# jacklu2016/or-gym-inventory

Measured on AMD Instinct MI355X. Metric: env-steps/sec (batched) at 1/2/4/8 MI355X; % HBM roofline, higher is better.
Workload: dtype int64

## Files before the change

or-gym-inventory_amd/csrc/capi.hip:

```cpp
#include <dlfcn.h>
#include <hip/hip_runtime.h>

#include <algorithm>
#include <cmath>
#include <cstdio>
#include <cstdlib>
#include <cstring>
#include <string>
#include <vector>

#include "../../include/invsim.h"
#include "kernels.hpp"

using namespace invsim;

namespace {

thread_local std::string g_last_error;

struct Field {
    std::string name;
    int64_t offset;
    int32_t elem;
    int32_t rows;
// ... 9 lines not shown
hipError_t ptrs_stats_nv_ph(unsigned long long *out, bool clear);
hipError_t ptrs_stats_im(unsigned long long *out, bool clear);
hipError_t ptrs_stats_im_ph(unsigned long long *out, bool clear);
hipError_t ptrs_stats_netspec(unsigned long long *out, bool clear);
hipError_t ptrs_stats_net(unsigned long long *out, bool clear);
#endif
}

struct invsim_handle {
    int32_t family = 0;
    int32_t device = 0;
    int64_t N = 0, Npad = 0;
    int32_t obs_dim = 0, act_dim = 0, demand_dim = 1;
    char *arena = nullptr;
    int64_t arena_bytes = 0;
    char *tables = nullptr;
    void *scratch = nullptr;
    bool la_valid = false;
    int la_slot = 0;
    std::vector<Field> fields;
    Common cm{};
    NvParams nv{};
    ImParams im{};
    NetParams net{};
    int32_t im_m1 = 0;
    bool im_backlog = false;
    int32_t net_spec = 0;
    bool t_known = true;
    int32_t t_cur = 0;
    int32_t horizon = 0;
    bool past_ok = false;
    int32_t demand_stream = INVSIM_DEMAND_NUMPY;
    uint64_t ph_step = 0;
    int64_t o_phstep = 0;
    bool ph_from_blob = false;
    bool capturing = false;
    bool cap_t_known = true, cap_la_valid = false;
    int32_t cap_t_cur = 0;
    int cap_la_slot = 0;
    int64_t cap_steps = 0;
    std::string err;
};

namespace {

struct Roctx {
// ... 207 lines not shown
        if (p && n) std::memcpy(b.data() + off, p, n * sizeof(T));
        return (int64_t)off;
    }
};

template <typename T>
const T *tab(invsim_handle *h, int64_t off) {
    return reinterpret_cast<const T *>(h->tables + off);
}

bool valid_autoreset(int32_t m) { return m >= 0 && m <= 2; }

int finish_create(invsim_handle *h, invsim_handle **out, int rc) {
    if (rc != INVSIM_OK) {
        g_last_error = h->err;
        invsim_destroy(h);
        *out = nullptr;
        return rc;
    }
    *out = h;
    return INVSIM_OK;
}

int64_t pad_n(int64_t n) { return std::max<int64_t>(256, (n + 255) / 256 * 256); }

void rhs_table(PtrsConst &c, std::vector<double> &tab) {
    c.k0 = 0;
    c.nk = 0;
    c.toff = (int32_t)tab.size();
    if (!(c.lam >= 10) || c.lam > 1e8) return;
    const double sd = std::sqrt(c.lam);
    int64_t k0 = std::max<int64_t>(0, (int64_t)std::floor(c.lam - 12 * sd - 10));
    const int64_t k1 = (int64_t)std::ceil(c.lam + 12 * sd + 40);
    int64_t n = k1 - k0;
    if (n > RHS_LDS_MAX) {
        k0 = std::max<int64_t>(0, (int64_t)std::floor(c.lam) - RHS_LDS_MAX / 2 + 20);
        n = RHS_LDS_MAX;
    }
    for (int64_t k = k0; k < k0 + n; k++)
        tab.push_back(-c.lam + (double)k * c.loglam - np_loggam((double)(k + 1)));
    c.k0 = (int32_t)k0;
    c.nk = (int32_t)n;
}

}

extern "C" {
// ... 164 lines not shown
        p.cm = h->cm;
        if (s->dist == 2) p.nd = np_dist_binomial(s->dist_n, s->dist_p);
        if (s->dist == 3) p.nd = np_dist_integers(s->dist_low, s->dist_high);
        if (s->dist == 4) p.nd = np_dist_geometric(s->dist_p);
        p.periods = s->periods;
        p.lt_max = D;
        p.dist = s->dist;
        int off = 0;
        for (int i = 0; i < m1; i++) {
            p.L[i] = (int32_t)s->lead_time[i];
            p.ring_off[i] = off;
            off += p.L[i];
            p.c[i] = s->supply_capacity[i];
            p.I0[i] = s->I0[i];
        }
        for (int j = 0; j < m; j++) {
            p.up[j] = (double)s->unit_price[j];
            p.uc[j] = (double)s->unit_cost[j];
            p.hc[j] = (double)s->holding_cost[j];
            p.kc[j] = (double)s->demand_cost[j];
        }
        p.pc = pc;
        p.alpha_pow = tab<double>(h, o_ap);
        p.user_D = tab<int64_t>(h, o_ud);
        p.I = at<int64_t>(h, o_I);
        p.B = at<int64_t>(h, o_B);
        p.Rring = at<int64_t>(h, o_R);
        p.alog = at<int64_t>(h, o_A);
        p.alog32 = at<uint32_t>(h, o_A32);
        p.ahead = nullptr;
        if (s->dist >= 1 && s->dist <= 4) {
            hipError_t e = hipMalloc(&h->scratch, (size_t)(2 * 4 * h->Npad * sizeof(uint64_t)));
            if (e != hipSuccess) rc = fail(h, INVSIM_ENOMEM, "hipMalloc(lookahead cache)");
            else p.ahead = static_cast<uint64_t *>(h->scratch);
        }
        if (rc == INVSIM_OK) rc = init_period(h, s->periods);
    }
    return finish_create(h, out, rc);
}

int invsim_create_netinvmgmt(const invsim_netinvmgmt_spec *s, int64_t n, int32_t device, int32_t ar,
                             invsim_handle **out) {
    if (!s || !out) return fail(nullptr, INVSIM_EINVAL, "null argument");
    if (n < 0 || n > (int64_t)1 << 31) return fail(nullptr, INVSIM_EINVAL, "n_envs out of range");
    if (!valid_autoreset(ar)) return fail(nullptr, INVSIM_EINVAL, "bad autoreset mode");
    const int J = s->n_main, E = s->n_reorder, RL = s->n_retail;
// ... 369 lines not shown
        for (int k = 0; k < K; k++) {
            if (t >= h->horizon && h->cm.autoreset == AR_DISABLED && !h->past_ok)
                return fail(h, INVSIM_ERANGE, "step past the episode horizon with autoreset disabled; reset first");
            t = next_period(t, h->horizon, h->cm.autoreset, h->past_ok);
        }
    }
    if (h->demand_stream == INVSIM_DEMAND_PHILOX) {
        int rc = ph_counter_sync(h, s);
        if (rc != INVSIM_OK) return rc;
    }
    if (h->cm.ep_ret && h->N && !reward)
        return fail(h, INVSIM_EINVAL, "the episode sink folds the reward outputs: pass reward / terminated / truncated");
    bool sunk = false;
    hipError_t e = hipSuccess;
    switch (h->family) {
        case INVSIM_NEWSVENDOR: {
            StepIO<float, float> io{K, (const float *)actions, (float *)obs, reward, terminated, truncated, (float *)final_obs};
            e = nv_run_launch(h->nv, t_u, pol, io, h->la_valid, h->la_slot, s);
            break;
        }
        case INVSIM_INVMGMT: {
            StepIO<int64_t, int64_t> io{K, (const int64_t *)actions, (int64_t *)obs, reward, terminated, truncated,
                                        (int64_t *)final_obs};
            e = im_run_launch(h->im, h->im_m1, h->im_backlog, t_u, pol, io, h->la_valid, h->la_slot, sunk, s);
            break;
        }
        case INVSIM_NETINVMGMT: {
            StepIO<float, float> io{K, (const float *)actions, (float *)obs, reward, terminated, truncated, (float *)final_obs};
            e = h->net_spec ? net_spec_launch(h->net_spec, h->net, t_u, pol, io, h->la_valid, h->la_slot, s)
                            : net_run_launch(h->net, t_u, pol, io, s);
            break;
        }
        default: return fail(h, INVSIM_EINVAL, "bad handle family");
    }
    if (e != hipSuccess) {
        h->la_valid = false;
        return hip_fail(h, e, "step launch");
    }
    if (h->cm.ep_ret && !sunk) {
        if (!reward) return fail(h, INVSIM_EINVAL, "the episode sink needs this launch's reward outputs");
        e = episode_fold_groups_launch(reward, terminated, truncated, K, h->N, h->cm.ep_ret, h->cm.ep_part, s);
        if (e != hipSuccess) return hip_fail(h, e, "episode sink fold");
    }
    if (h->demand_stream == INVSIM_DEMAND_PHILOX) h->ph_step += (uint64_t)K;
    if (h->t_known) {
        for (int k = 0; k < K; k++) h->t_cur = next_period(h->t_cur, h->horizon, h->cm.autoreset, h->past_ok);
    } else if (h->cm.autoreset == AR_DISABLED && !h->past_ok) {
// ... 308 lines not shown
```

or-gym-inventory_amd/csrc/invmgmt.hip:

```cpp
#include "kernels.hpp"

namespace invsim {
namespace {

#ifdef INVSIM_TIMING
__device__ uint64_t g_tbuf[TB_WAVES * TB_PROBES];
#endif

constexpr uint32_t IM_WIDE = 0xFFFFFFFFu;

__device__ __forceinline__ int64_t alog_get(const ImParams &P, int64_t idx) {
    const uint32_t v = P.alog32[idx];
    return v == IM_WIDE ? P.alog[idx] : (int64_t)v;
}

constexpr int im_wlane(int m1) { return m1 * (9 < 36 / m1 ? 9 : 36 / m1); }

__device__ __forceinline__ int64_t wrap_add(int64_t a, int64_t b) {
    return (int64_t)((uint64_t)a + (uint64_t)b);
}
__device__ __forceinline__ int64_t wrap_sub(int64_t a, int64_t b) {
    return (int64_t)((uint64_t)a - (uint64_t)b);
}

__device__ __forceinline__ int64_t min_via_f64(int64_t a, int64_t sup) {
    const double x = (double)a, y = (double)sup;
    return (int64_t)((x <= y) ? x : y);
}

// ... 447 lines not shown
    const int64_t S = P.cm.Npad;
    const int O = M1 * (P.lt_max + 1);
#pragma unroll
    for (int i = 0; i < M1; i++) P.I[i * S + e] = P.I0[i];
    if (BACKLOG) {
#pragma unroll
        for (int q = 0; q <= M1; q++) P.B[q * S + e] = 0;
    }
    P.cm.period[e] = 0;
    if (obs) {
        int64_t *orow = obs + e * O;
        for (int q = 0; q < O; q++) orow[q] = (q < M1) ? P.I0[q] : 0;
    }
}

__device__ __forceinline__ void wg_lds_sync() {
    TBAR_T0();
    __builtin_amdgcn_fence(__ATOMIC_RELEASE, "workgroup", "local");
    __builtin_amdgcn_s_barrier();
    __builtin_amdgcn_fence(__ATOMIC_ACQUIRE, "workgroup", "local");
    TBAR_ADD();
}

template <int M1, bool BACKLOG, bool NPD, bool AHEAD, class RG = Pcg>
__global__ void __launch_bounds__(2 * WAVE)
im_split_kernel(ImParams P, int t, StepIO<int64_t, int64_t> io, int cur, int la0, int gla) {
    extern __shared__ __attribute__((aligned(16))) int64_t im_tile[];
    const int64_t N = P.cm.N;
    const int64_t S = P.cm.Npad;
    double *rhs_l = reinterpret_cast<double *>(im_tile + (int64_t)WAVE * M1 * (P.lt_max + 1));
    uint64_t *Acur = P.ahead ? P.ahead + (int64_t)cur * 4 * S : nullptr;
    uint64_t *Anxt = P.ahead ? P.ahead + (int64_t)(cur ^ 1) * 4 * S : nullptr;
    const int64_t udem = P.user_D[t];
    auto stage_table = [&](int lane) {
        TableStage ts;
        ts.dst = rhs_l;
        const bool has_tab = P.pc.nk > 0 && P.dist == 1;
        const double *tsrc = has_tab ? P.rhs : P.alpha_pow;
        const int qm = has_tab ? P.pc.nk - 1 : 0;
#pragma unroll
        for (int u = 0; u < TableStage::NT; u++) ts.v[u] = tsrc[min(lane + u * WAVE, qm)];
        return ts;
    };
    auto draw = [&](auto &g, uint64_t &u32) -> int64_t {
#ifdef INVSIM_ABL_NO_POISSON
        int64_t x = 20 + (int64_t)(g.lo & 3);
        g.next64();
#else
        int64_t x = NPD ? np_demand(g, u32, P.nd) : (P.dist == 5) ? udem : env_poisson(g, P.pc, rhs_l);
#endif
        return x < 0 ? 0 : x;
    };
    constexpr bool DEC = AHEAD;
    const int bid = (int)blockIdx.x;
    TPROBE(0);
    TPROBE_ID();
    if (AHEAD && bid >= la0 && bid < la0 + gla) {
        const int64_t e = (int64_t)(bid - la0) * (2 * WAVE) + threadIdx.x;
        const bool valid = e < N;
        const int64_t ee = valid ? e : N - 1;
        TableStage ts = stage_table((int)(threadIdx.x & (WAVE - 1)));
        if constexpr (RG::kCounter) {
            RG g;
            P.cm.rng.load(ee, g);
            g.set_step(P.cm.ph_step + 1);
            g.sub(0);
            uint64_t u32 = 0;
            ts.flush((int)(threadIdx.x & (WAVE - 1)));
            const int64_t dn = draw(g, u32);
            if (valid) st_store(Anxt + 2 * S + e, (uint64_t)dn);
            return;
        }
        Pcg g;
        g.hi = Acur[ee];
        g.lo = Acur[S + ee];
        g.inc_hi = P.cm.rng.inc_hi[ee];
        g.inc_lo = P.cm.rng.inc_lo[ee];
        uint64_t u32 = NPD ? Acur[3 * S + ee] : 0;
        PtrsJumpLane jt;
        jt.load((int)(threadIdx.x & (WAVE - 1)));
        ts.flush((int)(threadIdx.x & (WAVE - 1)));
        TPROBE(1);
        int64_t dn;
#ifndef INVSIM_ABL_NO_POISSON
        if (!NPD && P.dist == 1 && P.pc.lam >= 10)
            dn = np_poisson_ptrs_compact(
                g, P.pc, RhsTab{rhs_l}, true, jt,
                [](const PtrsConst &c, int) { return c; });
        else
#endif
            dn = draw(g, u32);
        TPROBE(2);
        if (valid) {
            st_store(Anxt + e, g.hi);
            st_store(Anxt + S + e, g.lo);
            st_store(Anxt + 2 * S + e, (uint64_t)dn);
            if (NPD) st_store(Anxt + 3 * S + e, u32);
        }
        TWAIT();
        TPROBE(5);
        return;
    }
    const int lane = threadIdx.x & (WAVE - 1);
    const bool demand_wave = threadIdx.x < WAVE;
    const int64_t e0 = (int64_t)(AHEAD && bid >= la0 ? bid - gla : bid) * WAVE;
    const int64_t e = e0 + lane;
    const bool valid = e < N;
    const int nvalid = (int)((N - e0) < WAVE ? (N - e0) : WAVE);
    const int D = P.lt_max;
    const int O = M1 * (D + 1);
    int64_t *trow = im_tile + (int64_t)lane * O;
    int64_t *w = trow + M1;
    int64_t *dsh = reinterpret_cast<int64_t *>(rhs_l + RHS_LDS_MAX);
    const int t1 = t + 1;
    const int n = D > 0 ? (t1 < D ? t1 : D) : 0;
    const int nw = n > 0 ? (n - 1) * M1 : 0;
    const int64_t tcount = (int64_t)nvalid * O;
    const int64_t thalf = ((tcount / 2) + 1) & ~(int64_t)1;
    constexpr int WL = im_wlane(M1);
    const bool wreg = (D - 1) * M1 <= WL;
    const int slot0 = D > 0 ? (int)((uint32_t)(t1 - n) % (uint32_t)D) : 0;
    auto wrow = [&](int r) -> int64_t {
        int slot = slot0 + r;
        slot = slot >= D ? slot - D : slot;
        return ((int64_t)slot * S + e) * M1;
    };
#ifndef INVSIM_IM_SPLIT_RW
#define INVSIM_IM_SPLIT_RW 6
#endif
    constexpr int RWN = WL / M1;
    constexpr int RW = INVSIM_IM_SPLIT_RW < RWN ? INVSIM_IM_SPLIT_RW : RWN;
    constexpr int WD = (RWN - RW) * M1 > 0 ? (RWN - RW) * M1 : 1;
    const bool wsplit = DEC && wreg && RW < RWN;
    const int u_dyn = wsplit ? RW * M1 : WL;
    const int rmax = nw > 0 ? nw / M1 - 1 : 0;
    if (demand_wave) {
        const int64_t ee = valid ? e : N - 1;
        TableStage ts;
        RG g;
        uint64_t u32 = 0;
        int64_t d = 0;
        if (AHEAD) {
            if (!DEC) d = (int64_t)Acur[2 * S + ee];
        } else {
            ts = stage_table(lane);
            P.cm.rng.load(ee, g);
            g.set_step(P.cm.ph_step);
            g.sub(0);
            if (NPD && !RG::kCounter) u32 = P.cm.u32buf[ee];
        }
        uint32_t wv[WL];
        {
#pragma unroll
            for (int r = 0; r < RWN; r++) {
#ifdef INVSIM_ABL_NO_WINDOW
#pragma unroll
                for (int i = 0; i < M1; i++) wv[r * M1 + i] = (uint32_t)(r + i);
#else
                if (r < RW || !wsplit) {
                    const uint32_t *src = P.alog32 + wrow(r < rmax ? r : rmax);
#pragma unroll
                    for (int i = 0; i < M1; i++) wv[r * M1 + i] = src[i];
                } else {
#pragma unroll
                    for (int i = 0; i < M1; i++) wv[r * M1 + i] = 0;
                }
#endif
            }
        }
        if (!AHEAD) {
            ts.flush(lane);
            d = draw(g, u32);
        }
        if (!DEC) dsh[lane] = d;
        if (D > 0) {
            if (wreg) {
                bool wide = false;
#pragma unroll
                for (int u = 0; u < WL; u++) {
                    if (u < (D - 1) * M1 && !(u >= nw && u < nw + M1) && !(u >= u_dyn && u < nw))
                        w[u] = (u < nw) ? (int64_t)wv[u] : 0;
                    wide |= (u < nw) && (u < u_dyn) && wv[u] == IM_WIDE;
                }
// ... 7 lines not shown
            } else {
                for (int q = 0; q < nw; q++) w[q] = alog_get(P, wrow(q / M1) + q % M1);
                for (int q = n * M1; q < D * M1; q++) w[q] = 0;
            }
        }
        if (!DEC) wg_lds_sync();
        if (DEC) TWAIT();
        TPROBE(6);
        if constexpr (!RG::kCounter) {
            if (!AHEAD && valid) {
                if (Acur) {
                    st_store(Acur + e, g.hi);
                    st_store(Acur + S + e, g.lo);
                    if (NPD) st_store(Acur + 3 * S + e, u32);
                } else {
                    P.cm.rng.store_state(e, g);
                    if (NPD) P.cm.u32buf[e] = u32;
                }
            }
        }
        wg_lds_sync();
        store_tile<(M1 * 11 * WAVE * 8 / 2 + 16 * WAVE - 1) / (16 * WAVE)>(im_tile, io.obs + e0 * O,
                                                                          thalf < tcount ? thalf : tcount, lane);
        if (!AHEAD && Anxt) {
            if constexpr (RG::kCounter) {
                g.set_step(P.cm.ph_step + 1);
                g.sub(0);
                u32 = 0;
            }
            const int64_t dn = draw(g, u32);
            if (valid) {
                if constexpr (!RG::kCounter) {
                    st_store(Anxt + e, g.hi);
                    st_store(Anxt + S + e, g.lo);
                    if (NPD) st_store(Anxt + 3 * S + e, u32);
                }
                st_store(Anxt + 2 * S + e, (uint64_t)dn);
            }
        }
        TWAIT();
        TPROBE(5);
        return;
    }
    TPROBE_AT(3, WAVE);
    const double apow = P.alpha_pow[t];
    const int64_t *arow = io.act + (valid ? e : N - 1) * M1;
    double *const ep_part = P.cm.ep_ret ? P.cm.ep_part + 4 * (e0 / WAVE) : nullptr;
    EpPart epp;
    double ep_r = 0.0;
    if (ep_part) {
        epp.load(ep_part);
        ep_r = P.cm.ep_ret[valid ? e : N - 1];
    }
    int64_t req[M1], arr[M1], I[M1], B[M1 + 1];
    const int64_t d_ahead = DEC ? (int64_t)Acur[2 * S + (valid ? e : N - 1)] : 0;
    uint32_t wd[WD];
    if (wsplit) {
#pragma unroll
        for (int r = RW; r < RWN; r++) {
#ifdef INVSIM_ABL_NO_WINDOW
#pragma unroll
            for (int i = 0; i < M1; i++) wd[(r - RW) * M1 + i] = (uint32_t)(r + i);
#else
            const uint32_t *src = P.alog32 + wrow(r < rmax ? r : rmax);
#pragma unroll
            for (int i = 0; i < M1; i++) wd[(r - RW) * M1 + i] = src[i];
#endif
        }
    }
#pragma unroll
    for (int i = 0; i < M1; i++) req[i] = arow[i];
#pragma unroll
    for (int i = 0; i < M1; i++) {
        const int L = P.L[i];
        const int row = L > 0 ? P.ring_off[i] + (int)((uint32_t)t % (uint32_t)L) : 0;
        arr[i] = P.Rring[(int64_t)row * S + e];
        if (!(L > 0 && t >= L)) arr[i] = 0;
    }
#pragma unroll
    for (int i = 0; i < M1; i++) I[i] = P.I[i * S + e];
#pragma unroll
    for (int q = 0; q <= M1; q++) B[q] = BACKLOG ? P.B[q * S + e] : 0;
    int64_t ordreq[M1], R[M1], Icur[M1];
#pragma unroll
    for (int i = 0; i < M1; i++) req[i] = req[i] > 0 ? req[i] : 0;
#pragma unroll
    for (int i = 0; i < M1; i++) {
        ordreq[i] = wrap_add(req[i], B[i + 1]);
        const int64_t r = ordreq[i] < P.c[i] ? ordreq[i] : P.c[i];
        R[i] = (i + 1 < M1) ? min_via_f64(r, I[i + 1]) : (int64_t)(double)r;
    }
#pragma unroll
    for (int i = 0; i < M1; i++) Icur[i] = wrap_add(I[i], P.L[i] == 0 ? R[i] : arr[i]);
#pragma unroll
    for (int i = 1; i < M1; i++) Icur[i] = wrap_sub(Icur[i], R[i]);
    int64_t Sv[M1 + 1], U[M1 + 1];
#pragma unroll
    for (int i = 0; i < M1; i++) {
        Sv[i + 1] = R[i];
        U[i + 1] = wrap_sub(ordreq[i], R[i]);
    }
    if (!DEC) wg_lds_sync();
    if (DEC) TWAIT();
    TPROBE_AT(1, WAVE);
    const int64_t d = DEC ? d_ahead : dsh[lane];
// ... 45 lines not shown
            const double rev = np_sum<double>(M1 + 1, [&](int q) { return P.up[q] * (double)Sv[q]; });
            const double pro = np_sum<double>(M1 + 1, [&](int q) { return P.uc[q] * (double)Sv[q]; });
            const double hol = np_sum<double>(M1 + 1, [&](int q) {
                const int64_t inv = (q < M1) ? Icur[q] : 0;
                return P.hc[q] * (double)(inv > 0 ? inv : 0);
            });
            const double pen = np_sum<double>(M1 + 1, [&](int q) { return P.kc[q] * (double)U[q]; });
            rr[2 * (M1 + 1) + 0] = __double_as_longlong(profit);
            rr[2 * (M1 + 1) + 1] = __double_as_longlong(rev);
            rr[2 * (M1 + 1) + 2] = __double_as_longlong(pro);
            rr[2 * (M1 + 1) + 3] = __double_as_longlong(hol);
            rr[2 * (M1 + 1) + 4] = __double_as_longlong(pen);
        }
        ImPending<M1> pend;
#pragma unroll
        for (int i = 0; i < M1; i++) {
            pend.R[i] = R[i];
            pend.req[i] = req[i];
        }
        pend.t = t;
        im_flush_pending<M1>(P, pend, e);
        out_store(io.rew + e, reward);
        out_store(io.term + e, (uint8_t)0);
        out_store(io.trunc + e, (uint8_t)(t1 >= P.periods ? 1 : 0));
        if (P.cm.info_demand) P.cm.info_demand[e] = d;
#pragma unroll
        for (int i = 0; i < M1; i++) st_store(P.I + i * S + e, Icur[i]);
        if (BACKLOG) {
#pragma unroll
            for (int q = 0; q <= M1; q++) st_store(P.B + q * S + e, U[q]);
        }
    }
    if (ep_part) {
        EpLane a;
        if (valid) {
            a.r = ep_r;
            a.add(reward, t1 >= P.periods);
            P.cm.ep_ret[e] = a.r;
        }
        epp.flush(ep_part, a, t1 >= P.periods, lane);
    }
    TWAIT();
    TPROBE_AT(4, WAVE);
}

template <int CH, int RD, class RG>
__device__ __forceinline__ void im_stream_loop(const ImParams &P, RG &g, const double *rhs_l, int64_t *dbuf,
                                               int lane, int K, int nb, int t_start) {
    StreamPos<RG> pos(P.cm.ph_step);
    stream_flat_loop<CH, RD, 1>(
        K, nb, t_start, P.periods,
        [&](int j, int, int64_t &d) {
#ifdef INVSIM_ABL_ROLL_NO_DRAW
            d = 20;
            return true;
#else
            pos.at(g, j, 0);
            return np_poisson_try(g, P.pc, rhs_l, d);
#endif
        },
        [&](int slot, int, int64_t d) { dbuf[slot * WAVE + lane] = d < 0 ? 0 : d; });
}

// ... 719 lines not shown
    const bool two = three && g2 && (g3.x % 2) == 0;
    const dim3 g6(g3.x / 2);
    const int sub = p.cm.kn.im_roll_sub >= WAVE ? (int)std::min<int64_t>(p.cm.kn.im_roll_sub / WAVE, g3.x) : (int)g3.x;
#define R_(B, POL)                                                                                                    \
    do {                                                                                                              \
        if (two) hipLaunchKernelGGL((im_roll3o_kernel<1, 5, 10, B, POL, RG, 2>), g6, dim3(6 * WAVE), 2 * G3::lds(POL), s, p, t_u, io, pv); \
        else if (three) hipLaunchKernelGGL((im_roll3o_kernel<1, 5, 10, B, POL, RG>), g3, dim3(3 * WAVE), G3::lds(POL), s, p, t_u, io, pv); \
        else                                                                                                          \
            for (int g0 = 0; g0 < (int)g3.x; g0 += sub)                                                               \
                hipLaunchKernelGGL((im_roll3_kernel<1, 5, 10, B, POL, RG>), dim3(min(sub, (int)g3.x - g0)), dim3(2 * WAVE), \
                                   G::lds(), s, p, t_u, io, pv, g0);                                                  \
    } while (0)
    if (pol) {
        if (backlog) R_(true, true);
        else R_(false, true);
    } else {
        if (backlog) R_(true, false);
        else R_(false, false);
    }
#undef R_
    return hipGetLastError();
}

}

#define IM_DISPATCH(M1V, BL, LAUNCH)                                   \
    switch (M1V) {                                                     \
        case 1: if (BL) LAUNCH(1, true); else LAUNCH(1, false); break; \
        case 2: if (BL) LAUNCH(2, true); else LAUNCH(2, false); break; \
        case 3: if (BL) LAUNCH(3, true); else LAUNCH(3, false); break; \
        case 4: if (BL) LAUNCH(4, true); else LAUNCH(4, false); break; \
        case 5: if (BL) LAUNCH(5, true); else LAUNCH(5, false); break; \
        case 6: if (BL) LAUNCH(6, true); else LAUNCH(6, false); break; \
        case 7: if (BL) LAUNCH(7, true); else LAUNCH(7, false); break; \
        case 8: if (BL) LAUNCH(8, true); else LAUNCH(8, false); break; \
        default: return hipErrorInvalidValue;                          \
    }

#ifdef INVSIM_IM_FAST_TU
hipError_t im_run_launch_ph(const ImParams &p, int M1, bool backlog, int t_u, const PolicyIO *pol,
                            const StepIO<int64_t, int64_t> &io, bool &ahead, int &slot, bool &sunk, hipStream_t s) {
    sunk = im_sink_noop(p, t_u, pol, io);
    if (p.cm.N == 0 || io.K <= 0) return hipSuccess;
    const size_t lds = (size_t)EPW * M1 * (p.lt_max + 1) * sizeof(int64_t) + RHS_LDS_MAX * sizeof(double);
    const dim3 grid(grid_for(p.cm.N, EPW)), block(WAVE);
    PolicyIO none{};
    const PolicyIO &pv = pol ? *pol : none;
    const bool npd = p.dist >= 2 && p.dist <= 4;
    if (im_split_applies(p, t_u, pol, io)) {
        const size_t lds2 = lds + WAVE * sizeof(int64_t);
        ImParams q = p;
        if (!p.cm.kn.im_ahead) q.ahead = nullptr;
        const bool hit = ahead && q.ahead;
        const int gla = hit ? (int)grid_for(p.cm.N, 2 * WAVE) : 0;
        const dim3 grid2(grid.x + gla), block2(2 * WAVE);
        const int cur = slot;
        const int la0 = 0;
#define S_(M, B)                                                                                        \
    do {                                                                                                \
        if (npd) {                                                                                      \
            if (hit) hipLaunchKernelGGL((im_split_kernel<M, B, true, true, PhiloxGen>), grid2, block2, lds2, s, q, t_u, io, cur, la0, gla);  \
            else hipLaunchKernelGGL((im_split_kernel<M, B, true, false, PhiloxGen>), grid2, block2, lds2, s, q, t_u, io, cur, la0, gla);     \
        } else {                                                                                        \
            if (hit) hipLaunchKernelGGL((im_split_kernel<M, B, false, true, PhiloxGen>), grid2, block2, lds2, s, q, t_u, io, cur, la0, gla); \
            else hipLaunchKernelGGL((im_split_kernel<M, B, false, false, PhiloxGen>), grid2, block2, lds2, s, q, t_u, io, cur, la0, gla);    \
        }                                                                                               \
    } while (0)
        IM_DISPATCH(M1, backlog, S_)
#undef S_
        sunk = true;
        ahead = q.ahead != nullptr;
        if (ahead) slot ^= 1;
        return hipGetLastError();
    }
    ahead = false;
    if (im_roll_applies(p, M1, t_u, pol, io)) {
        sunk = true;
        return im_roll_launch<PhiloxGen>(p, backlog, t_u, pol, io, s);
    }
#define K_(M, B, TU, ONE, POL)                                                                          \
    do {                                                                                                \
        if (npd)                                                                                        \
            hipLaunchKernelGGL((im_run_kernel<M, B, TU, ONE, POL, true, PhiloxGen>), grid, block, lds, s, p, t_u, io, pv);  \
        else                                                                                            \
            hipLaunchKernelGGL((im_run_kernel<M, B, TU, ONE, POL, false, PhiloxGen>), grid, block, lds, s, p, t_u, io, pv); \
    } while (0)
#define L_(M, B)                                             \
    do {                                                     \
        if (pol) {                                           \
            if (t_u >= 0) K_(M, B, true, false, true);       \
            else K_(M, B, false, false, true);               \
        } else if (io.K == 1) {                              \
            if (t_u >= 0) K_(M, B, true, true, false);       \
            else K_(M, B, false, true, false);               \
        } else {                                             \
            if (t_u >= 0) K_(M, B, true, false, false);      \
            else K_(M, B, false, false, false);              \
        }                                                    \
    } while (0)
    IM_DISPATCH(M1, backlog, L_)
#undef L_
#undef K_
    return hipGetLastError();
}

INVSIM_PTRS_STATS_TU(im_ph)
#else
hipError_t im_run_launch(const ImParams &p, int M1, bool backlog, int t_u, const PolicyIO *pol,
                         const StepIO<int64_t, int64_t> &io, bool &ahead, int &slot, bool &sunk, hipStream_t s) {
    sunk = im_sink_noop(p, t_u, pol, io);
    if (p.cm.N == 0 || io.K <= 0) return hipSuccess;
    const size_t lds = (size_t)EPW * M1 * (p.lt_max + 1) * sizeof(int64_t) + RHS_LDS_MAX * sizeof(double);
    const dim3 grid(grid_for(p.cm.N, EPW)), block(WAVE);
    PolicyIO none{};
    const PolicyIO &pv = pol ? *pol : none;
    const bool npd = p.dist >= 2 && p.dist <= 4;
    const bool ph = p.cm.philox != 0;
    if (ph) return im_run_launch_ph(p, M1, backlog, t_u, pol, io, ahead, slot, sunk, s);
    if (im_split_applies(p, t_u, pol, io)) {
        const size_t lds2 = lds + WAVE * sizeof(int64_t);
        const dim3 block2(2 * WAVE);
        ImParams q = p;
        if (!p.cm.kn.im_ahead) q.ahead = nullptr;
        if (ahead && !q.ahead) {
            const hipError_t ce = im_commit_launch(p, slot, s);
            ahead = false;
            if (ce != hipSuccess) return ce;
        }
        const bool hit = ahead && q.ahead;
        const int gla = hit ? (int)grid_for(p.cm.N, 2 * WAVE) : 0;
        const dim3 grid2(grid.x + gla);
        const int cur = slot;
        const int la0 = 0;
#define S_(M, B)                                                                                        \
    do {                                                                                                \
        if (npd) {                                                                                      \
            if (hit) hipLaunchKernelGGL((im_split_kernel<M, B, true, true>), grid2, block2, lds2, s, q, t_u, io, cur, la0, gla);  \
            else hipLaunchKernelGGL((im_split_kernel<M, B, true, false>), grid2, block2, lds2, s, q, t_u, io, cur, la0, gla);     \
        } else {                                                                                        \
            if (hit) hipLaunchKernelGGL((im_split_kernel<M, B, false, true>), grid2, block2, lds2, s, q, t_u, io, cur, la0, gla); \
            else hipLaunchKernelGGL((im_split_kernel<M, B, false, false>), grid2, block2, lds2, s, q, t_u, io, cur, la0, gla);    \
        }                                                                                               \
    } while (0)
        IM_DISPATCH(M1, backlog, S_)
#undef S_
        sunk = true;
        if (q.ahead) {
            ahead = true;
            slot ^= 1;
        } else {
            ahead = false;
        }
        return hipGetLastError();
    }
    if (!(!pol && io.K == 1 && t_u >= p.periods) && ahead) {
        const hipError_t ce = im_commit_launch(p, slot, s);
        ahead = false;
        if (ce != hipSuccess) return ce;
    }
    if (im_roll_applies(p, M1, t_u, pol, io)) {
        sunk = true;
        return im_roll_launch<Pcg>(p, backlog, t_u, pol, io, s);
    }
#define K_(M, B, TU, ONE, POL)                                                                         \
// ... 27 lines not shown
    hipLaunchKernelGGL(im_commit_kernel, dim3(grid_for(p.cm.N, 256)), dim3(256), 0, s, p, slot ^ 1);
    return hipGetLastError();
}

hipError_t im_reset_launch(const ImParams &p, int M1, bool backlog, const uint8_t *mask,
                           int64_t *obs, hipStream_t s) {
    if (p.cm.N == 0) return hipSuccess;
    const dim3 grid(grid_for(p.cm.N, 256)), block(256);
#define L_(M, B) hipLaunchKernelGGL((im_reset_kernel<M, B>), grid, block, 0, s, p, mask, obs)
    IM_DISPATCH(M1, backlog, L_)
#undef L_
    return hipGetLastError();
}

INVSIM_PTRS_STATS_TU(im)
#endif

}

#if defined(INVSIM_TIMING) && !defined(INVSIM_IM_FAST_TU)
extern "C" int invsim_debug_timing(void *dst, int64_t bytes) {
    return (int)hipMemcpyFromSymbol(dst, HIP_SYMBOL(invsim::g_tbuf), (size_t)bytes, 0, hipMemcpyDeviceToHost);
}
extern "C" int invsim_debug_timing_bar(void *dst, int64_t bytes) {
    return (int)hipMemcpyFromSymbol(dst, HIP_SYMBOL(invsim::g_tbar), (size_t)bytes, 0, hipMemcpyDeviceToHost);
}
#endif
```

or-gym-inventory_amd/csrc/kernels.hpp:

```cpp
#pragma once
#include <hip/hip_runtime.h>
#include <stdint.h>

#include "device_common.hpp"
#include "group_rng.hpp"
#include "numpy_dists.hpp"

namespace invsim {

enum { AR_NEXT_STEP = 0, AR_SAME_STEP = 1, AR_DISABLED = 2 };

#ifdef INVSIM_TIMING
constexpr int TB_WAVES = 8192, TB_PROBES = 8;
#define TPROBE(i)                                                                              \
    do {                                                                                       \
        if (threadIdx.x == 0 && blockIdx.x < TB_WAVES)                                         \
            g_tbuf[blockIdx.x * TB_PROBES + (i)] = __builtin_amdgcn_s_memrealtime();           \
    } while (0)
#define TPROBE_ID()                                                                            \
    do {                                                                                       \
        if (threadIdx.x == 0 && blockIdx.x < TB_WAVES)                                         \
            g_tbuf[blockIdx.x * TB_PROBES + 7] =                                               \
                ((uint64_t)__builtin_amdgcn_s_getreg((31 << 11) | 20) << 32) |                 \
                (uint32_t)__builtin_amdgcn_s_getreg((31 << 11) | 4);                           \
    } while (0)
#define TPROBE_AT(i, tid)                                                                      \
    do {                                                                                       \
        if (threadIdx.x == (tid) && blockIdx.x < TB_WAVES)                                     \
            g_tbuf[blockIdx.x * TB_PROBES + (i)] = __builtin_amdgcn_s_memrealtime();           \
    } while (0)
#define TPROBE_W(i)                                                                            \
    do {                                                                                       \
        const unsigned tw_ = blockIdx.x * (blockDim.x / 64) + threadIdx.x / 64;                \
// ... 192 lines not shown
struct ImParams {
    Common cm;
    int32_t periods;
    int32_t lt_max;
    int32_t dist;
    NpDist nd;
    int32_t L[IM_MAX_M1];
    int32_t ring_off[IM_MAX_M1];
    int64_t c[IM_MAX_M1];
    int64_t I0[IM_MAX_M1];
    double up[IM_MAX_M1 + 1], uc[IM_MAX_M1 + 1], hc[IM_MAX_M1 + 1], kc[IM_MAX_M1 + 1];
    PtrsConst pc;
    const double *rhs;
    const double *alpha_pow;
    const int64_t *user_D;
    int64_t *I;
    int64_t *B;
    int64_t *Rring;
    uint32_t *alog32;
    int64_t *alog;
    uint64_t *ahead;
};

struct NetParams {
    Common cm;
    int32_t J, E, RL, T, backlog, sumL;
    const double *I0, *h, *C, *o, *v;
    const int32_t *is_factory, *is_retail;
    const int32_t *sup, *pur, *sup_is_factory, *L, *ring_off;
    const int32_t *win_off;
    const double *lp, *lg;
    const int32_t *rl_node, *rl_user;
    const double *rl_p, *rl_b;
    const PtrsConst *rl_pc;
    const int32_t *rl_dist;
    const NpDist *rl_nd;
    const double *rhs;
    const double *user_D;
    const int32_t *succ_ptr, *succ_kind, *succ_idx, *pred_ptr, *pred_idx;
    const double *alpha_pow;
    double *X;
    double *U;
    double *Y;
    double *Rring;
    uint64_t *ahead;
};
// ... 180 lines not shown
    }
}

hipError_t seed_range_launch(const Common &cm, uint64_t base_lo, uint64_t base_hi, int64_t first,
                             const uint8_t *mask, hipStream_t s);
hipError_t seed_words_launch(const Common &cm, const uint32_t *words, const int32_t *nwords,
                             const uint8_t *mask, hipStream_t s);
hipError_t period_fill_launch(const Common &cm, int32_t t, hipStream_t s);
hipError_t episode_fold_launch(const double *rew, const uint8_t *term, const uint8_t *trunc, int32_t K,
                               int64_t N, double *ret, double *acc, hipStream_t s);
hipError_t episode_fold_groups_launch(const double *rew, const uint8_t *term, const uint8_t *trunc, int32_t K,
                                      int64_t N, double *ret, double *part, hipStream_t s);
hipError_t episode_ret_reset_launch(double *ret, const uint8_t *mask, int64_t N, hipStream_t s);

hipError_t nv_reset_launch(const NvParams &p, const uint8_t *mask, float *obs, hipStream_t s);
hipError_t nv_run_launch(const NvParams &p, int t_u, const PolicyIO *pol, const StepIO<float, float> &io,
                         bool &ahead, int &slot, hipStream_t s);
hipError_t nv_commit_launch(const NvParams &p, int slot, hipStream_t s);
hipError_t nv_run_launch_ph(const NvParams &p, int t_u, const PolicyIO *pol, const StepIO<float, float> &io,
                            bool &ahead, int &slot, hipStream_t s);

hipError_t im_reset_launch(const ImParams &p, int M1, bool backlog, const uint8_t *mask,
                           int64_t *obs, hipStream_t s);
hipError_t im_run_launch(const ImParams &p, int M1, bool backlog, int t_u, const PolicyIO *pol,
                         const StepIO<int64_t, int64_t> &io, bool &ahead, int &slot, bool &sunk, hipStream_t s);
hipError_t im_run_launch_ph(const ImParams &p, int M1, bool backlog, int t_u, const PolicyIO *pol,
                            const StepIO<int64_t, int64_t> &io, bool &ahead, int &slot, bool &sunk, hipStream_t s);
hipError_t im_commit_launch(const ImParams &p, int slot, hipStream_t s);

enum { NET_SPEC_NONE = 0, NET_SPEC_DEFAULT = 1, NET_SPEC_CUSTOM = 2 };
hipError_t net_spec_launch(int which, const NetParams &p, int t_u, const PolicyIO *pol,
                           const StepIO<float, float> &io, bool &ahead, int &slot, hipStream_t s);
hipError_t net_commit_launch(const NetParams &p, int slot, hipStream_t s);
hipError_t net_reset_launch(const NetParams &p, const uint8_t *mask, float *obs, hipStream_t s);
hipError_t net_run_launch(const NetParams &p, int t_u, const PolicyIO *pol, const StepIO<float, float> &io,
                          hipStream_t s);
size_t net_lds_bytes(const NetParams &p);

}
```

Baseline: 8.190 billion.

## Precompute per-step split-kernel scalars on host and pass hot pointers as kernel arguments

Moves per-step scalar derivations (alpha power, window slot, row max, truncation flag, arrival rows) from the device to the host. For M1=3 they are packed into one 32-bit word, and the hot pointers (actions, I, B, ring, alog32, lookahead) are passed directly as kernel arguments. The goal is to avoid dependent scalar loads from the large ImParams struct and the alpha_pow table at kernel start, shortening the critical path of the small batched step. It also hoists the state loads ahead of the episode-sink loads, reorders the RNG state loads, adds a waves-per-EU occupancy hint for one configuration, and adds timing probes. The cost is a host copy of the alpha table, a limit that N fit in int32, and a larger kernel argument block.

Result: faster. 8.408 billion (median of 6 runs) (+2.7%).

```diff
diff --git a/or-gym-inventory_amd/csrc/capi.hip b/or-gym-inventory_amd/csrc/capi.hip
--- a/or-gym-inventory_amd/csrc/capi.hip
+++ b/or-gym-inventory_amd/csrc/capi.hip
@@ -55,6 +55,7 @@
     Common cm{};
     NvParams nv{};
     ImParams im{};
+    std::vector<double> im_ap;
     NetParams net{};
     int32_t im_m1 = 0;
     bool im_backlog = false;
@@ -308,7 +309,6 @@
     return INVSIM_OK;
 }
 
-int64_t pad_n(int64_t n) { return std::max<int64_t>(256, (n + 255) / 256 * 256); }
 
 void rhs_table(PtrsConst &c, std::vector<double> &tab) {
     c.k0 = 0;
@@ -519,6 +519,7 @@
         }
         p.pc = pc;
         p.alpha_pow = tab<double>(h, o_ap);
+        h->im_ap = ap;
         p.user_D = tab<int64_t>(h, o_ud);
         p.I = at<int64_t>(h, o_I);
         p.B = at<int64_t>(h, o_B);
@@ -934,7 +935,7 @@
         case INVSIM_INVMGMT: {
             StepIO<int64_t, int64_t> io{K, (const int64_t *)actions, (int64_t *)obs, reward, terminated, truncated,
                                         (int64_t *)final_obs};
-            e = im_run_launch(h->im, h->im_m1, h->im_backlog, t_u, pol, io, h->la_valid, h->la_slot, sunk, s);
+            e = im_run_launch(h->im, h->im_ap.data(), h->im_m1, h->im_backlog, t_u, pol, io, h->la_valid, h->la_slot, sunk, s);
             break;
         }
         case INVSIM_NETINVMGMT: {
diff --git a/or-gym-inventory_amd/csrc/invmgmt.hip b/or-gym-inventory_amd/csrc/invmgmt.hip
--- a/or-gym-inventory_amd/csrc/invmgmt.hip
+++ b/or-gym-inventory_amd/csrc/invmgmt.hip
@@ -5,6 +5,15 @@
 
 #ifdef INVSIM_TIMING
 __device__ uint64_t g_tbuf[TB_WAVES * TB_PROBES];
+__device__ uint64_t g_targ[TB_WAVES * 2];
+#define TPROBE_ARGS(col, tid, dep)                                                             \
+    do {                                                                                       \
+        asm volatile("" ::"s"(dep));                                                           \
+        if (threadIdx.x == (tid) && blockIdx.x < TB_WAVES)                                     \
+            g_targ[blockIdx.x * 2 + (col)] = __builtin_amdgcn_s_memrealtime();                 \
+    } while (0)
+#else
+#define TPROBE_ARGS(col, tid, dep) do {} while (0)
 #endif
 
 constexpr uint32_t IM_WIDE = 0xFFFFFFFFu;
@@ -498,16 +507,31 @@
     TBAR_ADD();
 }
 
+constexpr int im_split_waves(int m1, bool npd, bool ahead, bool counter) {
+    return (m1 == 2 && npd && ahead && !counter) ? 5 : 1;
+}
 template <int M1, bool BACKLOG, bool NPD, bool AHEAD, class RG = Pcg>
 __global__ void __launch_bounds__(2 * WAVE)
-im_split_kernel(ImParams P, int t, StepIO<int64_t, int64_t> io, int cur, int la0, int gla) {
+    __attribute__((amdgpu_waves_per_eu(im_split_waves(M1, NPD, AHEAD, RG::kCounter))))
+im_split_kernel(const int64_t *act, int64_t *Ip, int64_t *Bp, const int64_t *Rr, const uint32_t *a32, uint64_t *Acur,
+                int32_t n32, uint32_t hw, ImParams P, int t, StepIO<int64_t, int64_t> io, int cur, double apow,
+                int n, int nw, int trunc) {
     extern __shared__ __attribute__((aligned(16))) int64_t im_tile[];
-    const int64_t N = P.cm.N;
-    const int64_t S = P.cm.Npad;
-    double *rhs_l = reinterpret_cast<double *>(im_tile + (int64_t)WAVE * M1 * (P.lt_max + 1));
-    uint64_t *Acur = P.ahead ? P.ahead + (int64_t)cur * 4 * S : nullptr;
-    uint64_t *Anxt = P.ahead ? P.ahead + (int64_t)(cur ^ 1) * 4 * S : nullptr;
-    const int64_t udem = P.user_D[t];
+    const int64_t N = n32;
+    const int64_t S = pad_n(N);
+    const int la0 = 0;
+    const int gla = AHEAD ? (int)((n32 + 2 * WAVE - 1) / (2 * WAVE)) : 0;
+    const bool hot = M1 == ImHot::M1 && __builtin_expect(ImHot::packed(hw), 1);
+    const int D = hot ? ImHot::depth(hw) : P.lt_max;
+    const int slot0 = hot ? ImHot::slot0(hw) : D > 0 ? (int)((uint32_t)(t + 1 - n) % (uint32_t)D) : 0;
+    const int rmax = hot ? ImHot::rmax(hw) : nw > 0 ? nw / M1 - 1 : 0;
+    auto arrival_row = [&](int i) -> int {
+        if (hot) return ImHot::row(hw, i) == ImHot::NOARR ? -1 : ImHot::row(hw, i);
+        const int L = P.L[i];
+        return (L > 0 && t >= L) ? P.ring_off[i] + (int)((uint32_t)t % (uint32_t)L) : -1;
+    };
+    double *rhs_l = reinterpret_cast<double *>(im_tile + (int64_t)WAVE * M1 * (D + 1));
+    auto anxt = [&]() -> uint64_t * { return P.ahead ? P.ahead + (int64_t)(cur ^ 1) * 4 * S : nullptr; };
     auto stage_table = [&](int lane) {
         TableStage ts;
         ts.dst = rhs_l;
@@ -523,7 +547,7 @@
         int64_t x = 20 + (int64_t)(g.lo & 3);
         g.next64();
 #else
-        int64_t x = NPD ? np_demand(g, u32, P.nd) : (P.dist == 5) ? udem : env_poisson(g, P.pc, rhs_l);
+        int64_t x = NPD ? np_demand(g, u32, P.nd) : (P.dist == 5) ? P.user_D[t] : env_poisson(g, P.pc, rhs_l);
 #endif
         return x < 0 ? 0 : x;
     };
@@ -532,11 +556,13 @@
     TPROBE(0);
     TPROBE_ID();
     if (AHEAD && bid >= la0 && bid < la0 + gla) {
+        TPROBE_ARGS(0, 0, (int)N + gla);
         const int64_t e = (int64_t)(bid - la0) * (2 * WAVE) + threadIdx.x;
         const bool valid = e < N;
         const int64_t ee = valid ? e : N - 1;
-        TableStage ts = stage_table((int)(threadIdx.x & (WAVE - 1)));
+        TableStage ts;
         if constexpr (RG::kCounter) {
+            ts = stage_table((int)(threadIdx.x & (WAVE - 1)));
             RG g;
             P.cm.rng.load(ee, g);
             g.set_step(P.cm.ph_step + 1);
@@ -544,15 +570,16 @@
             uint64_t u32 = 0;
             ts.flush((int)(threadIdx.x & (WAVE - 1)));
             const int64_t dn = draw(g, u32);
-            if (valid) st_store(Anxt + 2 * S + e, (uint64_t)dn);
+            if (valid) st_store(anxt() + 2 * S + e, (uint64_t)dn);
             return;
         }
         Pcg g;
         g.hi = Acur[ee];
         g.lo = Acur[S + ee];
+        uint64_t u32 = NPD ? Acur[3 * S + ee] : 0;
+        ts = stage_table((int)(threadIdx.x & (WAVE - 1)));
         g.inc_hi = P.cm.rng.inc_hi[ee];
         g.inc_lo = P.cm.rng.inc_lo[ee];
-        uint64_t u32 = NPD ? Acur[3 * S + ee] : 0;
         PtrsJumpLane jt;
         jt.load((int)(threadIdx.x & (WAVE - 1)));
         ts.flush((int)(threadIdx.x & (WAVE - 1)));
@@ -568,6 +595,7 @@
             dn = draw(g, u32);
         TPROBE(2);
         if (valid) {
+            uint64_t *const Anxt = anxt();
             st_store(Anxt + e, g.hi);
             st_store(Anxt + S + e, g.lo);
             st_store(Anxt + 2 * S + e, (uint64_t)dn);
@@ -583,19 +611,14 @@
     const int64_t e = e0 + lane;
     const bool valid = e < N;
     const int nvalid = (int)((N - e0) < WAVE ? (N - e0) : WAVE);
-    const int D = P.lt_max;
     const int O = M1 * (D + 1);
     int64_t *trow = im_tile + (int64_t)lane * O;
     int64_t *w = trow + M1;
     int64_t *dsh = reinterpret_cast<int64_t *>(rhs_l + RHS_LDS_MAX);
-    const int t1 = t + 1;
-    const int n = D > 0 ? (t1 < D ? t1 : D) : 0;
-    const int nw = n > 0 ? (n - 1) * M1 : 0;
     const int64_t tcount = (int64_t)nvalid * O;
     const int64_t thalf = ((tcount / 2) + 1) & ~(int64_t)1;
     constexpr int WL = im_wlane(M1);
     const bool wreg = (D - 1) * M1 <= WL;
-    const int slot0 = D > 0 ? (int)((uint32_t)(t1 - n) % (uint32_t)D) : 0;
     auto wrow = [&](int r) -> int64_t {
         int slot = slot0 + r;
         slot = slot >= D ? slot - D : slot;
@@ -609,8 +632,8 @@
     constexpr int WD = (RWN - RW) * M1 > 0 ? (RWN - RW) * M1 : 1;
     const bool wsplit = DEC && wreg && RW < RWN;
     const int u_dyn = wsplit ? RW * M1 : WL;
-    const int rmax = nw > 0 ? nw / M1 - 1 : 0;
     if (demand_wave) {
+        TPROBE_ARGS(0, 0, (int)N + gla);
         const int64_t ee = valid ? e : N - 1;
         TableStage ts;
         RG g;
@@ -634,7 +657,7 @@
                 for (int i = 0; i < M1; i++) wv[r * M1 + i] = (uint32_t)(r + i);
 #else
                 if (r < RW || !wsplit) {
-                    const uint32_t *src = P.alog32 + wrow(r < rmax ? r : rmax);
+                    const uint32_t *src = a32 + wrow(r < rmax ? r : rmax);
 #pragma unroll
                     for (int i = 0; i < M1; i++) wv[r * M1 + i] = src[i];
                 } else {
@@ -688,6 +711,7 @@
         wg_lds_sync();
         store_tile<(M1 * 11 * WAVE * 8 / 2 + 16 * WAVE - 1) / (16 * WAVE)>(im_tile, io.obs + e0 * O,
                                                                           thalf < tcount ? thalf : tcount, lane);
+        uint64_t *const Anxt = AHEAD ? nullptr : anxt();
         if (!AHEAD && Anxt) {
             if constexpr (RG::kCounter) {
                 g.set_step(P.cm.ph_step + 1);
@@ -709,8 +733,37 @@
         return;
     }
     TPROBE_AT(3, WAVE);
-    const double apow = P.alpha_pow[t];
-    const int64_t *arow = io.act + (valid ? e : N - 1) * M1;
+    TPROBE_ARGS(1, WAVE, (int)N + gla);
+    const int64_t *arow = act + (valid ? e : N - 1) * M1;
+    int64_t req[M1], arr[M1], I[M1], B[M1 + 1];
+    const int64_t d_ahead = DEC ? (int64_t)Acur[2 * S + (valid ? e : N - 1)] : 0;
+    uint32_t wd[WD];
+    if (wsplit) {
+#pragma unroll
+        for (int r = RW; r < RWN; r++) {
+#ifdef INVSIM_ABL_NO_WINDOW
+#pragma unroll
+            for (int i = 0; i < M1; i++) wd[(r - RW) * M1 + i] = (uint32_t)(r + i);
+#else
+            const uint32_t *src = a32 + wrow(r < rmax ? r : rmax);
+#pragma unroll
+            for (int i = 0; i < M1; i++) wd[(r - RW) * M1 + i] = src[i];
+#endif
+        }
+    }
+#pragma unroll
+    for (int i = 0; i < M1; i++) req[i] = arow[i];
+#pragma unroll
+    for (int i = 0; i < M1; i++) {
+        const int row = arrival_row(i);
+        const bool none = row < 0;
+        arr[i] = Rr[(int64_t)(none ? 0 : row) * S + e];
+        if (none) arr[i] = 0;
+    }
+#pragma unroll
+    for (int i = 0; i < M1; i++) I[i] = Ip[i * S + e];
+#pragma unroll
+    for (int q = 0; q <= M1; q++) B[q] = BACKLOG ? Bp[q * S + e] : 0;
     double *const ep_part = P.cm.ep_ret ? P.cm.ep_part + 4 * (e0 / WAVE) : nullptr;
     EpPart epp;
     double ep_r = 0.0;
@@ -718,35 +771,6 @@
         epp.load(ep_part);
         ep_r = P.cm.ep_ret[valid ? e : N - 1];
     }
-    int64_t req[M1], arr[M1], I[M1], B[M1 + 1];
-    const int64_t d_ahead = DEC ? (int64_t)Acur[2 * S + (valid ? e : N - 1)] : 0;
-    uint32_t wd[WD];
-    if (wsplit) {
-#pragma unroll
-        for (int r = RW; r < RWN; r++) {
-#ifdef INVSIM_ABL_NO_WINDOW
-#pragma unroll
-            for (int i = 0; i < M1; i++) wd[(r - RW) * M1 + i] = (uint32_t)(r + i);
-#else
-            const uint32_t *src = P.alog32 + wrow(r < rmax ? r : rmax);
-#pragma unroll
-            for (int i = 0; i < M1; i++) wd[(r - RW) * M1 + i] = src[i];
-#endif
-        }
-    }
-#pragma unroll
-    for (int i = 0; i < M1; i++) req[i] = arow[i];
-#pragma unroll
-    for (int i = 0; i < M1; i++) {
-        const int L = P.L[i];
-        const int row = L > 0 ? P.ring_off[i] + (int)((uint32_t)t % (uint32_t)L) : 0;
-        arr[i] = P.Rring[(int64_t)row * S + e];
-        if (!(L > 0 && t >= L)) arr[i] = 0;
-    }
-#pragma unroll
-    for (int i = 0; i < M1; i++) I[i] = P.I[i * S + e];
-#pragma unroll
-    for (int q = 0; q <= M1; q++) B[q] = BACKLOG ? P.B[q * S + e] : 0;
     int64_t ordreq[M1], R[M1], Icur[M1];
 #pragma unroll
     for (int i = 0; i < M1; i++) req[i] = req[i] > 0 ? req[i] : 0;
@@ -838,23 +862,23 @@
         im_flush_pending<M1>(P, pend, e);
         out_store(io.rew + e, reward);
         out_store(io.term + e, (uint8_t)0);
-        out_store(io.trunc + e, (uint8_t)(t1 >= P.periods ? 1 : 0));
+        out_store(io.trunc + e, (uint8_t)(trunc ? 1 : 0));
         if (P.cm.info_demand) P.cm.info_demand[e] = d;
 #pragma unroll
-        for (int i = 0; i < M1; i++) st_store(P.I + i * S + e, Icur[i]);
+        for (int i = 0; i < M1; i++) st_store(Ip + i * S + e, Icur[i]);
         if (BACKLOG) {
 #pragma unroll
-            for (int q = 0; q <= M1; q++) st_store(P.B + q * S + e, U[q]);
+            for (int q = 0; q <= M1; q++) st_store(Bp + q * S + e, U[q]);
         }
     }
     if (ep_part) {
         EpLane a;
         if (valid) {
             a.r = ep_r;
-            a.add(reward, t1 >= P.periods);
+            a.add(reward, trunc != 0);
             P.cm.ep_ret[e] = a.r;
         }
-        epp.flush(ep_part, a, t1 >= P.periods, lane);
+        epp.flush(ep_part, a, trunc != 0, lane);
     }
     TWAIT();
     TPROBE_AT(4, WAVE);
@@ -1620,9 +1644,42 @@
     return hipGetLastError();
 }
 
-}
-
-#define IM_DISPATCH(M1V, BL, LAUNCH)                                   \
+struct ImSplitArgs {
+    int32_t n32;
+    uint32_t hw;
+    uint64_t *acur;
+    double apow;
+    int n, nw, trunc;
+};
+inline ImSplitArgs im_split_args(const ImParams &q, const double *ap_host, int M1, int t, int cur) {
+    ImSplitArgs a{};
+    a.n32 = (int32_t)q.cm.N;
+    a.acur = q.ahead ? q.ahead + (int64_t)cur * 4 * pad_n(q.cm.N) : nullptr;
+    a.apow = ap_host[t];
+    const int D = q.lt_max, t1 = t + 1;
+    a.n = D > 0 ? (t1 < D ? t1 : D) : 0;
+    a.nw = a.n > 0 ? (a.n - 1) * M1 : 0;
+    a.trunc = t1 >= q.periods ? 1 : 0;
+    int sumL = 0;
+    for (int i = 0; i < M1; i++) sumL += q.L[i];
+    if (M1 == ImHot::M1 && D <= 15 && sumL <= ImHot::NOARR) {
+        const uint32_t slot0 = D > 0 ? (uint32_t)(t1 - a.n) % (uint32_t)D : 0;
+        const uint32_t rmax = a.nw > 0 ? (uint32_t)(a.nw / M1 - 1) : 0;
+        uint32_t w = (1u << 31) | slot0 | (rmax << 4) | ((uint32_t)D << 8);
+        for (int i = 0; i < M1; i++) {
+            const int L = q.L[i];
+            const uint32_t row = (L > 0 && t >= L) ? (uint32_t)(q.ring_off[i] + t % L) : (uint32_t)ImHot::NOARR;
+            w |= row << (12 + 6 * i);
+        }
+        a.hw = w;
+    }
+    return a;
+}
+#define IM_SPLIT_ARGS io.act, q.I, q.B, q.Rring, q.alog32, ha.acur, ha.n32, ha.hw, q, t_u, io, cur, ha.apow, ha.n, ha.nw, ha.trunc
+
+}
+
+#define IM_DISPATCH(M1V, BL, LAUNCH)                                  \
     switch (M1V) {                                                     \
         case 1: if (BL) LAUNCH(1, true); else LAUNCH(1, false); break; \
         case 2: if (BL) LAUNCH(2, true); else LAUNCH(2, false); break; \
@@ -1636,7 +1693,7 @@
     }
 
 #ifdef INVSIM_IM_FAST_TU
-hipError_t im_run_launch_ph(const ImParams &p, int M1, bool backlog, int t_u, const PolicyIO *pol,
+hipError_t im_run_launch_ph(const ImParams &p, const double *ap_host, int M1, bool backlog, int t_u, const PolicyIO *pol,
                             const StepIO<int64_t, int64_t> &io, bool &ahead, int &slot, bool &sunk, hipStream_t s) {
     sunk = im_sink_noop(p, t_u, pol, io);
     if (p.cm.N == 0 || io.K <= 0) return hipSuccess;
@@ -1653,15 +1710,16 @@
         const int gla = hit ? (int)grid_for(p.cm.N, 2 * WAVE) : 0;
         const dim3 grid2(grid.x + gla), block2(2 * WAVE);
         const int cur = slot;
-        const int la0 = 0;
+        if (p.cm.N > INT32_MAX - 2 * WAVE) return hipErrorInvalidValue;
+        const ImSplitArgs ha = im_split_args(q, ap_host, M1, t_u, cur);
 #define S_(M, B)                                                                                        \
     do {                                                                                                \
         if (npd) {                                                                                      \
-            if (hit) hipLaunchKernelGGL((im_split_kernel<M, B, true, true, PhiloxGen>), grid2, block2, lds2, s, q, t_u, io, cur, la0, gla);  \
-            else hipLaunchKernelGGL((im_split_kernel<M, B, true, false, PhiloxGen>), grid2, block2, lds2, s, q, t_u, io, cur, la0, gla);     \
+            if (hit) hipLaunchKernelGGL((im_split_kernel<M, B, true, true, PhiloxGen>), grid2, block2, lds2, s, IM_SPLIT_ARGS);  \
+            else hipLaunchKernelGGL((im_split_kernel<M, B, true, false, PhiloxGen>), grid2, block2, lds2, s, IM_SPLIT_ARGS);     \
         } else {                                                                                        \
-            if (hit) hipLaunchKernelGGL((im_split_kernel<M, B, false, true, PhiloxGen>), grid2, block2, lds2, s, q, t_u, io, cur, la0, gla); \
-            else hipLaunchKernelGGL((im_split_kernel<M, B, false, false, PhiloxGen>), grid2, block2, lds2, s, q, t_u, io, cur, la0, gla);    \
+            if (hit) hipLaunchKernelGGL((im_split_kernel<M, B, false, true, PhiloxGen>), grid2, block2, lds2, s, IM_SPLIT_ARGS); \
+            else hipLaunchKernelGGL((im_split_kernel<M, B, false, false, PhiloxGen>), grid2, block2, lds2, s, IM_SPLIT_ARGS);    \
         }                                                                                               \
     } while (0)
         IM_DISPATCH(M1, backlog, S_)
@@ -1704,7 +1762,7 @@
 
 INVSIM_PTRS_STATS_TU(im_ph)
 #else
-hipError_t im_run_launch(const ImParams &p, int M1, bool backlog, int t_u, const PolicyIO *pol,
+hipError_t im_run_launch(const ImParams &p, const double *ap_host, int M1, bool backlog, int t_u, const PolicyIO *pol,
                          const StepIO<int64_t, int64_t> &io, bool &ahead, int &slot, bool &sunk, hipStream_t s) {
     sunk = im_sink_noop(p, t_u, pol, io);
     if (p.cm.N == 0 || io.K <= 0) return hipSuccess;
@@ -1714,7 +1772,7 @@
     const PolicyIO &pv = pol ? *pol : none;
     const bool npd = p.dist >= 2 && p.dist <= 4;
     const bool ph = p.cm.philox != 0;
-    if (ph) return im_run_launch_ph(p, M1, backlog, t_u, pol, io, ahead, slot, sunk, s);
+    if (ph) return im_run_launch_ph(p, ap_host, M1, backlog, t_u, pol, io, ahead, slot, sunk, s);
     if (im_split_applies(p, t_u, pol, io)) {
         const size_t lds2 = lds + WAVE * sizeof(int64_t);
         const dim3 block2(2 * WAVE);
@@ -1729,15 +1787,16 @@
         const int gla = hit ? (int)grid_for(p.cm.N, 2 * WAVE) : 0;
         const dim3 grid2(grid.x + gla);
         const int cur = slot;
-        const int la0 = 0;
+        if (p.cm.N > INT32_MAX - 2 * WAVE) return hipErrorInvalidValue;
+        const ImSplitArgs ha = im_split_args(q, ap_host, M1, t_u, cur);
 #define S_(M, B)                                                                                        \
     do {                                                                                                \
         if (npd) {                                                                                      \
-            if (hit) hipLaunchKernelGGL((im_split_kernel<M, B, true, true>), grid2, block2, lds2, s, q, t_u, io, cur, la0, gla);  \
-            else hipLaunchKernelGGL((im_split_kernel<M, B, true, false>), grid2, block2, lds2, s, q, t_u, io, cur, la0, gla);     \
+            if (hit) hipLaunchKernelGGL((im_split_kernel<M, B, true, true>), grid2, block2, lds2, s, IM_SPLIT_ARGS);  \
+            else hipLaunchKernelGGL((im_split_kernel<M, B, true, false>), grid2, block2, lds2, s, IM_SPLIT_ARGS);     \
         } else {                                                                                        \
-            if (hit) hipLaunchKernelGGL((im_split_kernel<M, B, false, true>), grid2, block2, lds2, s, q, t_u, io, cur, la0, gla); \
-            else hipLaunchKernelGGL((im_split_kernel<M, B, false, false>), grid2, block2, lds2, s, q, t_u, io, cur, la0, gla);    \
+            if (hit) hipLaunchKernelGGL((im_split_kernel<M, B, false, true>), grid2, block2, lds2, s, IM_SPLIT_ARGS); \
+            else hipLaunchKernelGGL((im_split_kernel<M, B, false, false>), grid2, block2, lds2, s, IM_SPLIT_ARGS);    \
         }                                                                                               \
     } while (0)
         IM_DISPATCH(M1, backlog, S_)
@@ -1811,6 +1870,9 @@
 extern "C" int invsim_debug_timing(void *dst, int64_t bytes) {
     return (int)hipMemcpyFromSymbol(dst, HIP_SYMBOL(invsim::g_tbuf), (size_t)bytes, 0, hipMemcpyDeviceToHost);
 }
+extern "C" int invsim_debug_timing_args(void *dst, int64_t bytes) {
+    return (int)hipMemcpyFromSymbol(dst, HIP_SYMBOL(invsim::g_targ), (size_t)bytes, 0, hipMemcpyDeviceToHost);
+}
 extern "C" int invsim_debug_timing_bar(void *dst, int64_t bytes) {
     return (int)hipMemcpyFromSymbol(dst, HIP_SYMBOL(invsim::g_tbar), (size_t)bytes, 0, hipMemcpyDeviceToHost);
 }
diff --git a/or-gym-inventory_amd/csrc/kernels.hpp b/or-gym-inventory_amd/csrc/kernels.hpp
--- a/or-gym-inventory_amd/csrc/kernels.hpp
+++ b/or-gym-inventory_amd/csrc/kernels.hpp
@@ -9,6 +9,10 @@
 namespace invsim {
 
 enum { AR_NEXT_STEP = 0, AR_SAME_STEP = 1, AR_DISABLED = 2 };
+
+__host__ __device__ constexpr int64_t pad_n(int64_t n) {
+    return n <= 256 ? 256 : (n + 255) / 256 * 256;
+}
 
 #ifdef INVSIM_TIMING
 constexpr int TB_WAVES = 8192, TB_PROBES = 8;
@@ -247,6 +251,17 @@
     uint64_t *ahead;
 };
 
+constexpr int IM_HOT_DWORDS = 14;
+struct ImHot {
+    static constexpr int M1 = 3;
+    static constexpr int NOARR = 63;
+    __host__ __device__ static constexpr bool packed(uint32_t w) { return (w >> 31) != 0; }
+    __host__ __device__ static constexpr int slot0(uint32_t w) { return (int)(w & 15u); }
+    __host__ __device__ static constexpr int rmax(uint32_t w) { return (int)((w >> 4) & 15u); }
+    __host__ __device__ static constexpr int depth(uint32_t w) { return (int)((w >> 8) & 15u); }
+    __host__ __device__ static constexpr int row(uint32_t w, int i) { return (int)((w >> (12 + 6 * i)) & 63u); }
+};
+
 struct NetParams {
     Common cm;
     int32_t J, E, RL, T, backlog, sumL;
@@ -473,9 +488,9 @@
 
 hipError_t im_reset_launch(const ImParams &p, int M1, bool backlog, const uint8_t *mask,
                            int64_t *obs, hipStream_t s);
-hipError_t im_run_launch(const ImParams &p, int M1, bool backlog, int t_u, const PolicyIO *pol,
+hipError_t im_run_launch(const ImParams &p, const double *ap_host, int M1, bool backlog, int t_u, const PolicyIO *pol,
                          const StepIO<int64_t, int64_t> &io, bool &ahead, int &slot, bool &sunk, hipStream_t s);
-hipError_t im_run_launch_ph(const ImParams &p, int M1, bool backlog, int t_u, const PolicyIO *pol,
+hipError_t im_run_launch_ph(const ImParams &p, const double *ap_host, int M1, bool backlog, int t_u, const PolicyIO *pol,
                             const StepIO<int64_t, int64_t> &io, bool &ahead, int &slot, bool &sunk, hipStream_t s);
 hipError_t im_commit_launch(const ImParams &p, int slot, hipStream_t s);
 
```
